# m-hamza-mughal/RAG-Gesture

Hardware: AMD Instinct MI355X
Metric: SMPL-X frames/sec, len150 DDIM-50 + insertion guidance; 1/2/4/8 GPU (higher is better)
Workload: dtype bf16

## Files before the change

include/rg_gesture.h:

```cpp
#ifndef RG_GESTURE_H
#define RG_GESTURE_H

#include <stdint.h>

#ifdef __cplusplus
extern "C" {
#endif

typedef struct rg_handle rg_handle;

enum rg_status {
  RG_OK = 0,
  RG_ERR_INVALID = -1,
  RG_ERR_HIP = -2,
  RG_ERR_NO_DEVICE = -3
};

#define RG_VERSION 127
int rg_version(void);
int rg_create(rg_handle** out, int device);
void rg_destroy(rg_handle* h);
const char* rg_last_error(rg_handle* h);
int rg_num_cus(rg_handle* h);

int rg_ddim_update(rg_handle* h, const float* x, const float* x0, float* x_out, int64_t n,
                   float c_recip, float c_recipm1, float c_a, float c_b, void* stream);

int rg_cfg_ddim_update(rg_handle* h, const float* out, const float* x, float* x_out, float* x0_out,
                       const float* js, int B, int T, int D, float w_c, float w_u,
                       float c_recip, float c_recipm1, float c_a, float c_b, void* stream);
int rg_cfg_ddim_update_rows(rg_handle* h, const float* out_cond, const float* out_uncond, const float* x, float* x_out,
                            float* x_out2, const float* js, int B, int T, int D, float w_c, float w_u,
                            float c_recip, float c_recipm1, float c_a, float c_b, void* stream);

int rg_cfg_ddpm_update(rg_handle* h, const float* out, const float* x, const float* noise, float* x_out,
                       const float* js, int B, int T, int D, float w_c, float w_u, float c1, float c2, float sigma,
                       void* stream);

typedef struct rg_glue_args {
  const float* out_c_a;
  const float* out_u_a;
// ... 159 lines not shown
  const float* tbias;
  const float* src_mask;
  const float* qmask;
  float* head;
  float* dump;
  float* xbuf;
  void* gbuf;
  const int* form;
  int L, B, T, S;
  int step, step_b, split;
  int dump_stage, dump_layer;
  int pairs;
  int twin;
  int* glue_ctr;
  rg_glue_args glue;
} rg_seq_args;

int rg_seq_forward(rg_handle* h, const rg_seq_args* args_host, void* stream);
int rg_seq2_forward(rg_handle* h, const rg_seq_args* args_host, void* stream);

#define RG_SEQ_MANY_MAX 8
int rg_seq_forward_many(rg_handle* h, const rg_seq_args* const* args_host, int n, void* stream);

#define RG_LANE_STRIDE 32
int rg_seqx_forward(rg_handle* h, const rg_seq_args* args_host, void* stream);
int rg_lane_form(rg_handle* h, int* state, int lane, int nlanes, int narrow_wgs, int wide_wgs, int budget, void* stream);

typedef struct rg_venc_args {
  const void* wstream;
  const void* pstream;
  const float* x;
  float* out;
  float* xbuf;
  float* dump;
  int nseq, S, nb, dump_block;
  const int* post_rows;
  float* post_mu;
  float* post_logvar;
  int post_nrows, pad_;
} rg_venc_args;

int rg_venc_forward(rg_handle* h, const rg_venc_args* args_host, void* stream);
int rg_venc_forward_grouped(rg_handle* h, const rg_venc_args* args_host, int n, void* stream);

typedef struct rg_vdec_args {
  const void* wstream;
// ... 473 lines not shown
```

rag-gesture_amd/csrc/rg_seq2.hip:

```cpp
#if !defined(RG_SEQ_BODY_ONLY) && !defined(RG2_PACK_TWO)
#define RG_PACK2_ONE
#endif
#include "rg_common.h"
#include "rg_stationary.h"
#include "rg_tail.h"
#include "rg_seq_host.h"

namespace {

constexpr int RD = 6;
constexpr int UPL = RG_SEQ_UPL;
constexpr int PANEL = TP * 1024;
constexpr int OFF_RING = 2 * PANEL;
constexpr int NSEG_COND = 36, NSEG_UNC = 19, NSEG_TWIN = 34;
constexpr int NSEG_MAX = NSEG_COND > NSEG_TWIN ? NSEG_COND : NSEG_TWIN;
constexpr int MAX_SEG = 8 * NSEG_MAX + 5;
constexpr int OFF_DESC = OFF_RING + NW * RD * 1024;
constexpr int OFF_STAT = OFF_DESC + ((MAX_SEG * 8 + 15) & ~15);
constexpr int STAT_HALF = 2 * NW * TP * 2;
constexpr int LDS_BYTES = OFF_STAT + 2 * STAT_HALF * 4;
static_assert(LDS_BYTES <= 160 * 1024, "LDS budget");

#define U(name) U_##name = RG_SEQ_U_##name
enum { U(KV), U(KV2), U(Q), U(SAO), U(MIXX), U(Q3_0), U(MIX_0), U(Q3_1), U(MIX_1), U(Q3_2), U(MIX_2), U(FF1_0), U(FF2_0), U(FF1_1), U(FF2_1), U(FFO) };
// ... 31 lines not shown
#else
#define TLOG()
#endif

typedef std::integral_constant<int, 3> SeqBoth;
typedef std::integral_constant<int, 1> SeqFirst;
typedef std::integral_constant<int, 2> SeqSecond;

typedef f32x4 Acc2[2][4][3];
typedef u32x2 Held[2][4][3];

__device__ __forceinline__ void zero(Acc2& a) {
#pragma unroll
  for (int q = 0; q < 2; ++q)
#pragma unroll
    for (int j = 0; j < 4; ++j)
#pragma unroll
      for (int tb = 0; tb < 3; ++tb) a[q][j][tb] = f32x4{0.f, 0.f, 0.f, 0.f};
}

}

template <bool TWIN>
__device__ __forceinline__ void run_pair(const rg_seq_args& a, const int sA, const int sB, unsigned char* const smem) {
  float* const sStat = reinterpret_cast<float*>(smem + OFF_STAT);
  int tid_ = threadIdx.x;
  asm volatile("" : "+v"(tid_));
  const int tid = tid_, lane0 = tid & 63;
  const int wave = __builtin_amdgcn_readfirstlane(tid >> 6);
  unsigned char* const ring = smem + OFF_RING + wave * (RD * 1024);
  const int T = a.T, B = a.B, L = a.L, R = 2 * a.B;
  const bool cond = sA < B;
  const int seqs[2] = {sA, sB};
  const int clips[2] = {cond ? sA : sA - B, (cond && !TWIN) ? sB : sB - B};
  const int st = clips[0] >= a.split ? a.step_b : a.step;
#ifdef RG_STAMPS
  unsigned long long tacc[12] = {0, 0, 0, 0, 0, 0, 0, 0, 0, 0, 0, 0};
  int ncall = 0;
  const unsigned long long tk0 = __builtin_amdgcn_s_memrealtime();
#endif
  auto barx = [&]() {
    TSTART();
    bar();
    TSTOP(2);
  };
  const int NU = UPL * L + 2;
  const int nspl = TWIN ? NSEG_TWIN : cond ? NSEG_COND : NSEG_UNC;
// ... 75 lines not shown
          u32x4{pack2(v0[0], v0[1]), pack2(v0[2], v0[3]), pack2(v1[0], v1[1]), pack2(v1[2], v1[3])};
    }
  __syncthreads();

  rg_cursor<RD, rg_desc8> cur(ring, smem + OFF_DESC, wave, lane0);
  auto ring_wait = [&]() { wait_vmcnt<RD - 1>(); };
  auto consume = [&]() -> const unsigned char* {
#ifdef RG_STAMPS
    const unsigned long long tc0_ = __builtin_amdgcn_s_memrealtime();
    ring_wait();
    tacc[7] += __builtin_amdgcn_s_memrealtime() - tc0_;
#else
    ring_wait();
#endif
    return ring + cur.head * 1024;
  };
  cur.load_seg();
#pragma unroll
  for (int s = 0; s < RD; ++s) cur.issue(s);
#ifdef RG_STAMPS
  tacc[10] = __builtin_amdgcn_s_memrealtime() - tk0;
#endif

  float* const Rw = a.xbuf + ((size_t)blockIdx.x * 2 * NW + wave) * (12 * 64 * 4);
  unsigned char* const Gw = reinterpret_cast<unsigned char*>(a.gbuf) + (size_t)blockIdx.x * (8 * PANEL);
  auto store_R = [&](const Acc2& v) {
    LANE_LOCAL();
    TSTART();
#pragma unroll
    for (int q = 0; q < 2; ++q)
#pragma unroll
      for (int j = 0; j < 4; ++j)
#pragma unroll
        for (int tb = 0; tb < 3; ++tb)
          *reinterpret_cast<f32x4*>(Rw + ((size_t)(q * NW * 12 + j * 3 + tb) * 64 + lane) * 4) = v[q][j][tb];
    TSTOP(6);
  };
  auto load_R = [&](Acc2& v) {
    LANE_LOCAL();
    TSTART();
#pragma unroll
    for (int q = 0; q < 2; ++q)
#pragma unroll
      for (int j = 0; j < 4; ++j)
#pragma unroll
        for (int tb = 0; tb < 3; ++tb)
          v[q][j][tb] = *reinterpret_cast<const f32x4*>(Rw + ((size_t)(q * NW * 12 + j * 3 + tb) * 64 + lane) * 4);
    TSTOP(6);
// ... 692 lines not shown
  const int npc = ((split + 1) >> 1) + ((B - split + 1) >> 1);
  return pairs ? npc : 2 * npc;
}
__device__ __forceinline__ void seq2_block(const rg_seq_args& a, const int block, unsigned char* const smem) {
  const int B = a.B, split = min(max(a.split, 0), B);
  const int npc = ((split + 1) >> 1) + ((B - split + 1) >> 1);
  int p = block, kind0 = 0;
  if (!a.pairs) {
    if ((npc & 3) == 0) {
      const int x = block & 7, q = block >> 3;
      kind0 = x >= 4;
      p = 4 * q + (x & 3);
    } else {
      kind0 = block >= npc;
      p = block - kind0 * npc;
    }
  }
  int c0, c1;
  pair_clips(p, split, B, c0, c1);
  const int npass = a.pairs ? 2 : 1;
#pragma unroll 1
  for (int pass = 0; pass < npass; ++pass) {
    const int kind = a.pairs ? pass : kind0;
    run_pair<false>(a, c0 + kind * B, c1 + kind * B, smem);
    __syncthreads();
    int* const ctr = rg_tail::late_ctr();
    if (ctr && !a.dump_stage)
      rg_tail::arrive_and_glue<NTH>(ctr, c0, c1, reinterpret_cast<int*>(smem), __builtin_amdgcn_readfirstlane(threadIdx.x >> 6));
  }
}

#ifndef RG_SEQ_BODY_ONLY
__global__ void __launch_bounds__(NTH) rg_seq2_kernel(const rg_seq_args a) {
  extern __shared__ __attribute__((aligned(16))) unsigned char smem[];
#ifndef RG2_SHARE_SIMD
  RG_OWN_THE_SIMD();
#endif
  seq2_block(a, blockIdx.x, smem);
}

__global__ void __launch_bounds__(NTH) rg_seq2_twin_kernel(const rg_seq_args a) {
  extern __shared__ __attribute__((aligned(16))) unsigned char smem[];
#ifndef RG2_SHARE_SIMD
  RG_OWN_THE_SIMD();
#endif
  const int clip = blockIdx.x;
  run_pair<true>(a, clip, clip + a.B, smem);
  __syncthreads();
  if (rg_tail::late_ctr() && !a.dump_stage) rg_tail::glue_own<NTH>(clip, __builtin_amdgcn_readfirstlane(threadIdx.x >> 6));
}

extern "C" int rg_seq2_forward(rg_handle* h, const rg_seq_args* args_host, void* stream) {
  const std::string why = rg_seq_refusal(RG_SEQ2_ENTRY, args_host);
  if (!why.empty()) { if (h) h->err = why; return RG_ERR_INVALID; }
  const rg_seq_args& a = *args_host;
  static rg_attr_once lds_once, lds_once_twin;
  if (a.twin) { RG_RESERVE_LDS(h, lds_once_twin, rg_seq2_twin_kernel, LDS_BYTES); }
  else { RG_RESERVE_LDS(h, lds_once, rg_seq2_kernel, LDS_BYTES); }
  rg_prof_scope prof(h, stream, 3, rg_seq_flops(a));
  if (a.twin) hipLaunchKernelGGL(rg_seq2_twin_kernel, dim3(a.B), dim3(NTH), LDS_BYTES, rg_stream(stream), a);
  else hipLaunchKernelGGL(rg_seq2_kernel, dim3(seq2_grid(a.B, a.split, a.pairs)), dim3(NTH), LDS_BYTES, rg_stream(stream), a);
  RG_CHECK_LAUNCH(h);
  prof.stop();
  return RG_OK;
}
#endif
```

rag-gesture_amd/csrc/rg_seq_host.h:

```cpp
#pragma once
#include <string>

#include "../../include/rg_gesture.h"

struct rg_seq_entry { const char *name, *need_bufs, *need_form, *no_dump, *twin_range, *twin_pairs, *no_twin; };
constexpr rg_seq_entry RG_SEQ_ENTRY = {"rg_seq_forward", nullptr, nullptr, nullptr, nullptr, nullptr, nullptr};
constexpr rg_seq_entry RG_SEQ2_ENTRY = {"rg_seq2_forward", "the two-sequence forward needs its scratch buffers xbuf and gbuf", nullptr,
                                        nullptr, "twin must be 0 or 1", "twin and pairs are two launch forms: set one of them", nullptr};
constexpr rg_seq_entry RG_SEQX_ENTRY = {
    "rg_seqx_forward", "the two-sequence form needs its scratch buffers xbuf and gbuf", "form: the lane's flag (rg_lane_form) must be given",
    "diagnostic dumps: use rg_seq_forward / rg_seq2_forward", nullptr, nullptr,
    "the twin form (one clip per workgroup) is not one of the device-chosen forms: use rg_seq2_forward"};

inline bool rg_seq_glue_ok(const rg_seq_args& a) {
  if (!a.glue_ctr) return true;
  const rg_glue_args& g = a.glue;
  if (a.dump_stage || g.n_a < 0 || g.n_b < 0 || g.n_a + g.n_b != a.B || g.T != a.T || g.D != 512 || !g.js || g.g_iter_next < 0) return false;
  if (g.n_a && !(g.out_c_a && g.out_u_a && g.x_a)) return false;
  if (g.n_b && !(g.out_c_b && g.out_u_b && g.x_b)) return false;
  return !g.in_seq_next || g.noise_next;
}

inline std::string rg_seq_refusal(const rg_seq_entry& e, const rg_seq_args* args) {
  const char* why = nullptr;
// ... 16 lines not shown
  }
  return why ? std::string(e.name) + ": " + why : std::string();
}

constexpr rg_seq_entry RG_SEQ_MANY_ENTRY = {"rg_seq_forward_many", nullptr, nullptr, "diagnostic dumps: use rg_seq_forward", nullptr, nullptr,
                                            "the twin form is rg_seq2_forward's: a grouped launch runs one workgroup per sequence"};

inline std::string rg_seq_many_refusal(const rg_seq_args* const* args, const int n) {
  const std::string name = std::string(RG_SEQ_MANY_ENTRY.name) + ": ";
  if (!args || n < 1) return name + "null or empty list of sessions";
  if (n > RG_SEQ_MANY_MAX) return name + "too many sessions (at most RG_SEQ_MANY_MAX)";
  for (int i = 0; i < n; ++i) {
    const std::string why = rg_seq_refusal(RG_SEQ_MANY_ENTRY, args[i]);
    if (!why.empty()) return why;
    const rg_seq_args &a = *args[i], &a0 = *args[0];
    if (a.pairs) return name + "pairs is another launch form: a grouped launch runs one workgroup per sequence";
    if (!(a.L == a0.L && a.T == a0.T && a.S == a0.S)) return name + "the sessions must agree in L, T and S";
    if (!(a.wstream == a0.wstream && a.pstream == a0.pstream && a.ustream == a0.ustream))
      return name + "the sessions must share the weight, parameter and table streams";
  }
  return std::string();
}

inline double rg_seq_flops(const rg_seq_args& a) {
  const double unit = 2.0 * a.T * 512 * 512, att = 2.0 * a.T * 32 * 32 * 16;
  const double cond = (RG_SEQ_UPL * a.L + 2) * unit + a.L * (2 + 3) * att, unc = (10 * a.L + 2) * unit + a.L * 2 * att;
  return a.B * (cond + unc);
}
```

rag-gesture_amd/csrc/rg_tail.h:

```cpp
#pragma once
#include "rg_common.h"
#include <cstddef>

namespace rg_tail {

typedef __attribute__((ext_vector_type(4))) float f32x4;
typedef __attribute__((ext_vector_type(4))) unsigned u32x4;
constexpr int COHERENT = 17;

__device__ __forceinline__ float ddim_one(float x, float x0, float c_recip, float c_recipm1, float c_a, float c_b) {
#pragma clang fp contract(off)
  float eps = (c_recip * x - x0) / c_recipm1;
  return x0 * c_a + c_b * eps;
}
__device__ __forceinline__ float cfg_one(float oc, float ou, float jc, float ju, float w_c, float w_u) {
#pragma clang fp contract(off)
  return oc * w_c * jc + ou * w_u * ju;
}

template <typename P>
__device__ __forceinline__ P* uniform_ptr(P* p) {
  const unsigned long long v = reinterpret_cast<unsigned long long>(p);
  return reinterpret_cast<P*>((unsigned long long)__builtin_amdgcn_readfirstlane((unsigned)(v >> 32)) << 32 |
                              (unsigned)__builtin_amdgcn_readfirstlane((unsigned)v));
// ... 153 lines not shown
  if (wave == 0 && lane == 0) {
    int m = 0;
    if (__hip_atomic_fetch_add(ctr + c0, 1, __ATOMIC_RELAXED, __HIP_MEMORY_SCOPE_AGENT) & 1) m |= 1;
    if (c1 != c0 && (__hip_atomic_fetch_add(ctr + c1, 1, __ATOMIC_RELAXED, __HIP_MEMORY_SCOPE_AGENT) & 1)) m |= 2;
    *flag = m;
  }
  __syncthreads();
  const int m = *flag;
  __syncthreads();
  if (m == 0) return;
  const rg_glue_args g = late_arg<rg_glue_args>(base + offsetof(rg_seq_args, glue));
  const float ton = two_over_numel(g);
#pragma unroll 1
  for (int q = 0; q < 2; ++q) {
    if (!(m >> q & 1)) continue;
    const int c = q ? c1 : c0;
    const bool ga = c < g.n_a;
    const int cl = ga ? c : c - g.n_a;
    glue_clip<NTH / 64>(g, ga, cl, wave, lane, ton);
  }
}

template <int NTH>
__device__ __forceinline__ void glue_own(const int c, const int wave) {
  const int lane = __builtin_amdgcn_mbcnt_hi(~0u, __builtin_amdgcn_mbcnt_lo(~0u, 0u));
  const rg_glue_args g = late_arg<rg_glue_args>(offsetof(rg_seq_args, glue));
  const bool ga = c < g.n_a;
  glue_clip<NTH / 64>(g, ga, ga ? c : c - g.n_a, wave, lane, two_over_numel(g));
}
}
```

rag-gesture_amd/denoiser.py:

```python
import math

import numpy as np
import torch

from . import capi, gemm as G, seqfwd as SQ

CONDS = ("xf_text", "xf_audio", "xf_spk")
BLOCKS = ("sa_block", "ca_blocks.xf_text", "ca_blocks.xf_audio", "ca_blocks.xf_spk", "ffn")


def _timestep_embedding(timesteps, dim, max_period=10000):
    half = dim // 2
    freqs = torch.exp(-math.log(max_period) * torch.arange(0, half, dtype=torch.float32) / half)
    args = timesteps[:, None].float() * freqs[None]
    return torch.cat([torch.cos(args), torch.sin(args)], dim=-1)


class DenoiserWeights:

    KV_GROUP = 2

    @staticmethod
    def _fold_ln(W, b, gamma, beta, pw, f32):
        Wp = (W.double() * gamma.double()[None, :]).float()
# ... 322 lines not shown
    def chain_end(self):
        if self.sq is not None:
            self.sq.chain_end()

    def forward(self, x, step, step_b=None, split=None, glue=None):
        w, h, B, R, M, D, T = self.w, self.h, self.B, self.R, self.M, self.w.D, self.w.T
        if split is not None and not (0 < split < B):
            step, step_b, split = (step if split >= B else step_b), None, None
        if self.sq is not None:
            if glue is not None and not x.is_contiguous():
                raise capi.RgError("DenoiserSession.forward(glue=...): x is updated in place and must be contiguous")
            return self.sq.run(x.contiguous(), step, step_b, split, glue=glue)
        if glue is not None:
            raise capi.RgError("DenoiserSession.forward(glue=...): the sequence-stationary engine only")
        if self.ln_mode == "auto":
            out = self._forward_guarded(x, step)
            if split is None:
                return out
        return self._forward_chain(x, step, step_b, split)

    @staticmethod
    def forward_many(sessions, calls):
        for s, kw in zip(sessions, calls):
            if s.sq is None or not kw["x"].is_contiguous():
                raise capi.RgError("DenoiserSession.forward_many: the sequence-stationary engine only, x contiguous")
        return SQ.run_many([s.sq for s in sessions], calls)

    LN_GUARD_SIGMAS = 3.0

    def _forward_guarded(self, x, step):
        if torch.cuda.is_current_stream_capturing():
            raise capi.RgError("DenoiserSession(ln_mode='auto'): run one forward before capturing a graph")
        self._guard = torch.zeros(1, device=self.w.dev)
        self.ln_mode = "folded"
        out = self._forward_chain(x, step)
        self.ln_ratio = float(self._guard.item())
        self._guard = None
        if self.ln_ratio > self.LN_GUARD_SIGMAS ** 2:
            self.ln_mode, self.xa_bf = "prologue", None
            out = self._forward_chain(x, step)
        return out

    def _guard_stats(self, stats):
        if getattr(self, "_guard", None) is not None:
            self.h.call("ln_guard", stats, self.M, stats.shape[1], self.w.D, self._guard)

# ... 118 lines not shown
```

rag-gesture_amd/pipeline.py:

```python
import collections
import ctypes
import contextlib
import copy
import os
import time
import types

import torch
import yaml

from . import capi, denoiser, sampler, schedule as sched_mod, seqfwd, vae as vae_mod

MODELS = {}


def register_module(cls):
    MODELS[cls.__name__] = cls
    return cls


def register_with_mmcv(force=False):
    regs = []
    try:
        from mmcv.cnn import MODELS as mmcv_models
# ... 42 lines not shown
        "step_increasing_from_25": list(range(steps - 1, -1, -1))[:half] + [0] * half,
        "decreasing_till_25": [0] * half + list(range(half)),
        "increasing_from_25": list(range(half - 1, -1, -1)) + [0] * half,
    }
    if name not in table:
        raise ValueError("Invalid guidance_iters value")
    return table[name]


E_BUCKET = 4


def bucket(n, m=None):
    m = E_BUCKET if m is None else m
    return -(-n // m) * m


def pad_rows(t, n):
    return t if t.shape[0] == n else torch.cat([t, t[:1].expand(n - t.shape[0], *t.shape[1:])], dim=0)


def lane_rows(t, dim, b0, b1):
    return None if t is None else (t[b0:b1] if dim == 0 else t[:, b0:b1])


def exemplar_query_masks(qmask, clips, n):
    return {c: pad_rows(torch.stack([qmask[b] for b in clips]), n) for c in denoiser.CONDS}


class _TorchNoise:
    order_free = True

    def __init__(self, device, generator=None):
        self.device, self.generator = device, generator

    def draw(self, shape, device=None):
        return torch.randn(*shape, device=self.device, generator=self.generator)


def draw_batch_noise(tape, dev, B, T, D, S, use_inversion, use_insertion_guidance, visualize_inversion, ddpm, has_in_seq, n_exemplars):
    x = tape.draw((B, T, D)).to(dev).contiguous()
    start_noise = x if use_inversion else None
    invl = torch.zeros(S, B, T, D, device=dev) if use_inversion and use_insertion_guidance else None
    ddpm_noise = inseq_noise = None
    if use_inversion and visualize_inversion and not isinstance(tape, _TorchNoise):
        for _ in range(S * sum(n_exemplars[:B])):
# ... 166 lines not shown
        return {k: copy.deepcopy(v, memo) for k, v in dict.items(self) if k not in self._PLAIN}

    def __reduce__(self):
        self._ready()
        return (dict, (), None, None, iter([(k, v) for k, v in dict.items(self) if k not in self._PLAIN]))


@register_module
class MotionDiffusion(torch.nn.Module):

    profile_phases = False
    rotation_lanes = None
    form_lanes = None
    _cur_rot = None
    _last_state = None

    def __init__(self, model=None, loss_recon=None, loss_gen=None, loss_contact=None, loss_laplace=None,
                 diffusion_train=None, diffusion_test=None, init_cfg=None, inference_type="ddpm",
                 genloss_acceleration_weight=True, genloss_hands_weight=2, genloss_smooth=True,
                 body_part_lossweights=None, device="cuda", precision="bf16", lanes=2, sample_lanes=None, session_options=None,
                 vae_options=None, async_results=False, slots=2, max_inflight=2, cobatch_lanes="batch", base_lanes=8,
                 batch_lanes=4, lane_streams=None, calibrate_lanes=True, decode_stream=False, dynamic_forms=False, dynamic_budget=None, invert_alone_wide=True, tail_glue=True,
                 cache_exemplar_latents=True, exemplar_cache_bytes=8 << 30, skip_clip_encode=True, grouped_decode=True,
                 grouped_drain=True, **kwargs):
        super().__init__()
        self.grouped_drain = bool(grouped_drain)
        self.grouped_decode = bool(grouped_decode)
        self.cache_exemplar_latents, self.exemplar_cache_bytes = bool(cache_exemplar_latents), int(exemplar_cache_bytes)
        self.skip_clip_encode = bool(skip_clip_encode)
        self.model = build_submodule(model, device=device, **kwargs)
        dt = dict(diffusion_test)
        self.schedule = sched_mod.Schedule(beta_scheduler=dt["beta_scheduler"], diffusion_steps=dt["diffusion_steps"],
                                           respace=dt.get("respace"))
        capi.require(dt.get("model_mean_type", "start_x") == "start_x" and dt.get("classifier_free_guidance_scale", 0) == 0,
                "unsupported argument: requires dt.get(\"model_mean_type\", \"start_x\") == \"start_x\" and dt.get(\"classifier_free_guidance_scale\", 0) == 0")
        self.inference_type = inference_type
        capi.require(inference_type in ("ddim", "ddpm"), "inference_type is 'ddim' (shipped config) or 'ddpm'")
        self.device, self.precision = torch.device(device), precision
        self.training = False
        self.session_options, self.vae_options = dict(session_options or {}), dict(vae_options or {})
        self.vae_options.setdefault("grouped_decode", self.grouped_decode)
        self._state = None
        self._sessions = {}
        self._graphs = {}
        self.use_graphs = True
        self.graph_captures = self.graph_cross_stream_waits = 0
        self._jitter = None
        self.phase_ms = {}
# ... 356 lines not shown
        motion_mask = gre.latent_mask(kwargs["motion_mask"].float())
        T = motion_mask.shape[1]
        n_lat = (T - 3) // 4
        up_i, ha_i, fa_i, lt_i = (list(range(0, n_lat)), list(range(n_lat + 1, 2 * n_lat + 1)),
                                  list(range(2 * n_lat + 2, 3 * n_lat + 2)), list(range(3 * n_lat + 3, T)))
        qmask = torch.ones_like(motion_mask)
        for r in ((T - 3) // 4, 2 * (T - 3) // 4, 3 * (T - 3) // 4):
            qmask[:, r] = 0
        query_masks = {c: qmask for c in denoiser.CONDS}

        plan = self._lane_plan(B)
        plan_s = self._lane_plan(B, self.sample_lanes)
        main = torch.cuda.current_stream()
        run_async = self.async_results and self.slots > 1 and not self.profile_phases
        cob = self._cob if run_async else None
        pid = None
        if cob is not None and cob.get("lane") is not None:
            self._lane_plan(B)
            n_rot = self.rotation_lanes or (self.batch_lanes if use_inversion else self.base_lanes)
            n_rot = max(1, min(int(n_rot), len(self._lane_streams)))
            self._cur_rot = self.form_lanes or n_rot
            pid = cob["lane"] % n_rot
            plan = plan_s = [(pid, self._lane_streams[pid], 0, B)]
        if run_async:
            self._slot = self._take_slot(pid, main, self._lanes_of(plan, plan_s))
        else:
            self._slot = 0
            self._wait_slot(main, self._lanes_of(plan, plan_s), 0)
        gre.concurrent_parts(not run_async and not self.use_graphs)
        word, audio, spk = kwargs["word"], kwargs["audio"], kwargs["speaker_ids"]
        with self._phase("conditions"):
            for lane, stream, b0, b1 in ([] if cob is not None else plan_s):
                cstream = main if run_async else stream
                cstream.wait_stream(main)
                with torch.cuda.stream(cstream):
                    self._sample_conditions(lane, b0, b1, word, audio, spk, motion_mask, qmask)
        with self._phase("vae_encode"):
            if self.skip_clip_encode and not self.training:
                tr_rel = gre.relative_trans(kwargs["motion_upper"], kwargs["motion_lower"], kwargs["motion_face"],
                                            kwargs["motion_hands"], f(kwargs["trans"]))
                capi.require(4 * (kwargs["motion_upper"].shape[1] // gre.frame_chunk_size) + 3 == T,
                             "unsupported argument: requires motion.shape[1] == T")
            else:
                motion, tr_rel = gre.encode_device_graphed(
                    f(kwargs["motion_upper"]), f(kwargs["motion_lower"]), f(kwargs["motion_face"]), f(kwargs["motion_hands"]),
                    f(kwargs["trans"]), f(kwargs["facial"]), f(kwargs["contact"]), [f(e) for e in eps_list])
                capi.require(motion.shape[1] == T, "unsupported argument: requires motion.shape[1] == T")
# ... 127 lines not shown

    def flush(self):
        cob, self._cob = self._cob, dict(lane=0)
        try:
            self._finish_pending()
        finally:
            self._cob = cob
        out = list(self._ready)
        self._ready.clear()
        return out

    def _finish_alone(self, st):
        main = st.main = torch.cuda.current_stream()
        st.slot = self._take_slot(st.pid, main, self._lanes_of(st.plan_s))
        for lane, stream, b0, b1 in st.plan_s:
            self._sample_conditions(lane, b0, b1, st.word, st.audio, st.spk, st.motion_mask, st.qmask)
        self._sampling_pass(st)
        return self._tail(st)

    def _pending_upto(self, seq):
        return sorted((p for p in self._pend if self._pend[p].seq <= seq), key=lambda p: self._pend[p].seq)

    def _finish_pending(self, upto=None, resume=None):
        sts = [self._pend.pop(p) for p in self._pending_upto(float("inf") if upto is None else upto)]
        group = self._drain_group(sts) if self.grouped_drain else []
        if group:
            self._drain_grouped(group)
        for st in sts:
            self._ready.append(self._tail(st) if any(st is g for g in group) else self._finish_alone(st))
        if resume is not None:
            self._slot = self._slots[resume.pid] = resume.slot

    DRAIN_SLOT = 0

    def _drain_group(self, sts):
        sett = lambda st: (st.T, st.S, bool(st.use_insertion_guidance), tuple(int(v) for v in st.guidance_iters), float(st.guidance_lr))

        def alone_on_a_lane(st):
            return (st.run_async and st.via_submit and not st.ddpm and st.prev_future is None and st.plan == st.plan_s
                    and len(st.plan_s) == 1 and tuple(st.plan_s[0][2:]) == (0, st.B))

        def one_sequence_form(st):
            o = self._session_opts(st.B, "sample", st.plan_s[0][0])
            return (self._runs_seq_engine(o) and not o.get("seq_pairs") and not o.get("seq_duo") and not o["seq_twin"] and "lane_dyn" not in o
                    and o["tail_glue"] and sampler.TAIL_GLUE and self.model.weights.h.recorder is None)
        if self.precision != "bf16":
# ... 46 lines not shown
        ins = {}
        for tag, (word, audio, spk, mask, qm) in (("a", a), ("b", b)):
            ins["word_" + tag], ins["audio_" + tag] = word.to(dev).float(), audio.to(dev).float()
            ins["spk_" + tag], ins["mask_" + tag] = spk.to(dev).long(), mask.to(dev).float()
            for c in denoiser.CONDS:
                ins["q_%s_%s" % (c, tag)] = qm[c].to(dev).float()

        def run(st):
            for tag, off, fin in (("a", 0, False), ("b", n_a, True)):
                sess.set_conditions(st["word_" + tag], st["audio_" + tag], st["spk_" + tag], st["mask_" + tag],
                                    {c: st["q_%s_%s" % (c, tag)] for c in denoiser.CONDS}, offset=off, finalize=fin)
            return ()
        self._graph_run(key + tuple(tuple(v.shape) for v in ins.values()), ins, run, owner=own)

    def _submit_chain(self, st):
        pend, S, T, D, dev = self._pend.get(st.pid), st.S, st.T, st.D, self.device
        lanes = [(lane, stream, b0, b1, self._exemplars(st, b0, b1)) for lane, stream, b0, b1 in st.plan] if st.use_inversion else []
        so = self.session_options
        groups_ok = self.precision == "bf16" and (self._runs_seq_engine(so) or so.get("styl_prepass", True))
        can_defer = (groups_ok and st.use_inversion and not st.visualize_inversion and not st.ddpm and st.plan == st.plan_s
                     and all(ex for *_, ex in lanes))
        same = pend is not None and can_defer and (pend.B, pend.T) == (st.B, st.T) and \
            [(b0, b1) for _, _, b0, b1 in pend.plan] == [(b0, b1) for _, _, b0, b1 in st.plan]
        if pend is not None and not same:
            self._finish_pending(pend.seq, resume=st)
            pend = None
        if not can_defer:
            self._finish_pending(resume=st)
            for lane, stream, b0, b1 in st.plan_s:
                self._sample_conditions(lane, b0, b1, st.word, st.audio, st.spk, st.motion_mask, st.qmask)
            self._inversion_pass(st)
            self._sampling_pass(st)
            self._ready.append(self._tail(st))
            return None
        if pend is None:
            self._inversion_pass(st)
            for lane, stream, _, _ in st.plan:
                self._slot_done[(lane, st.slot)] = [stream.record_event()]
            self._pend[st.pid] = st
            return None
        main = st.main
        self._fill_prev(pend, main)
        guided = pend.use_insertion_guidance
        gi, lr = tuple(int(v) for v in pend.guidance_iters), float(pend.guidance_lr)
        work = []
        for lane, stream, b0, b1, ex in lanes:
            Bl = b1 - b0
            Ep, cat = self._exemplar_inputs(st, ex, main)
            okey = (Bl + Ep, "cobatch", lane, self._slot)
            sess = self._session(Bl + Ep, "cobatch", lane)
            eqm = exemplar_query_masks(st.qmask, [b for b, _ in ex], Ep)
            self._set_conditions_pair(
                sess, ("cond2", Bl, Ep, lane, self._slot), okey,
                (pend.word[b0:b1], pend.audio[b0:b1], pend.spk[b0:b1], pend.motion_mask[b0:b1], {c: pend.qmask[b0:b1] for c in denoiser.CONDS}),
                (cat("retr_text"), cat("retr_audio"), cat("retr_spkid"), cat("retr_motion_mask"), eqm), Bl)
            work.append((lane, stream, b0, b1, ex, Ep, sess, okey, cat("retr_motion_latent").float().contiguous()))
        for lane, stream, b0, b1, ex, Ep, sess, okey, x_e in work:
            Bl = b1 - b0
            stream.wait_stream(main)
            self._used_on(stream, pend.x, pend.in_seq, pend.inseq_noise, pend.invl, pend.x_out, x_e, st.start_noise, st.invl, st.qmask)
            with torch.cuda.stream(stream):
                sl = lambda t, dim: lane_rows(t, dim, b0, b1)
                ins = dict(xa=sl(pend.x, 0), in_seq=sl(pend.in_seq, 0), noise=sl(pend.inseq_noise, 1),
                           invl=sl(pend.invl, 1) if guided else None, xb=x_e)

                def loop(s, sess=sess, Bl=Bl, Ep=Ep):
                    x_all = torch.cat([s["xa"], s["xb"]], dim=0).contiguous()
                    out_b = torch.empty(S, Ep, T, D, device=dev)
                    sampler.cobatched_loop(sess, x_all, Bl, out_b, inverted_a=s["invl"], guidance_iters=gi, guidance_lr=lr,
                                           inseq_noise_a=s["noise"], in_seq_a=s["in_seq"], tail_glue=self.tail_glue)
                    return x_all[:Bl], out_b
                key = ("cobatch", Bl, Ep, lane, T, self._slot, guided, pend.in_seq is not None, gi, lr, self.tail_glue)
                xl, inv = self._graph_run(key, ins, loop, owner=okey)
                pend.x_out[b0:b1].copy_(xl)
                self._splice(st, ex, inv, Ep)
                self._zero_prev_rows(st, b0, b1)
        pend.main, pend.slot = main, self._slot
        self._ready.append(self._tail(pend))
        self._pend[st.pid] = st
        return None

    def _exemplars(self, st, b0, b1):
        return [(b, q) for b in range(b0, b1) for q in st.retrieval_dict["retr_uncropped_latents"][b].keys()]

    def _exemplar_inputs(self, st, ex, stream):
        dev = self.device
        Ep = bucket(len(ex))
        lat = lambda b, q: st.retrieval_dict["retr_uncropped_latents"][b][q]

        def cat(key):
            parts = [lat(b, q)[key].to(dev) for b, q in ex]
            self._used_on(stream, *parts)
            return pad_rows(torch.cat(parts, dim=0), Ep)
        return Ep, cat

    def _splice(self, st, ex, inv, Ep):
        h, rd = self.model.weights.h, st.retrieval_dict
        lvl = st.inversion_start_time % st.S
        rows = []
        for e, (b, q_idx) in enumerate(ex):
            r0, r1 = rd["retr_startends"][b][q_idx]
            q0, q1 = rd["query_startends"][b][q_idx]
            capi.require(r1 - r0 == q1 - q0, "unsupported argument: requires r1 - r0 == q1 - q0")
# ... 136 lines not shown
```

rag-gesture_amd/sampler.py:

```python
import ctypes

import torch

from . import capi

from .seqfwd import GlueArgs, MANY_MAX

SPLICE_MAX = capi.header_constants()["RG_SPLICE_MAX"]
SpliceTable = capi.struct("rg_splice_table")


TAIL_GLUE = True


def _tail_ok(sess, x):
    return (TAIL_GLUE and getattr(sess, "tail_glue", True) and getattr(sess, "sq", None) is not None and sess.h.recorder is None and x.is_cuda and x.is_contiguous()
            and x.dtype == torch.float32 and x.shape[0] == sess.B)


def _p(t):
    if t is None:
        return None
    if not (t.is_cuda and t.is_contiguous() and t.dtype == torch.float32):
        raise capi.RgError("rg_cobatch_glue: contiguous fp32 device tensors expected")
# ... 138 lines not shown
        tail = bool(tail_glue) and _tail_ok(sess, x_all) and 0 < n_a < B
        for k in range(S):
            i = S - 1 - k
            if not tail:
                sess.forward(x_all, i, step_b=k, split=n_a)
            nxt = None if i == 0 else (inverted_a[i - 1] if inverted_a is not None else in_seq_a)
            a = _glue(sess, guidance_lr, i=i, x_a=xa, n_a=n_a, nxt=nxt, noise_nxt=None if nxt is None else inseq_noise_a[i - 1],
                      g_next=guidance_iters[i - 1] if inverted_a is not None and i > 0 else 0, k=k, x_b=xb, keep_b=out_b[k], n_b=n_b)
            if tail:
                sess.forward(x_all, i, step_b=k, split=n_a, glue=a)
            else:
                h.call("cobatch_glue", ctypes.byref(a))
        sess.chain_end()
        return x_all, out_b
    for k in range(S):
        i, g_iter = S - 1 - k, None
        if inverted_a is not None and i != S - 1:
            in_seq, g_iter = inverted_a[i], guidance_iters[i]
        _step(sess, xa, i, in_seq, None if in_seq is None else inseq_noise_a[i], g_iter, guidance_lr, n_a, (x_all, k, xb, out_b[k]))
    sess.chain_end()
    return x_all, out_b


class GraphedLoop:

    def __init__(self, fn, warmup=True):
        if warmup:
            s = torch.cuda.Stream()
            s.wait_stream(torch.cuda.current_stream())
            with torch.cuda.stream(s):
                fn()
            torch.cuda.current_stream().wait_stream(s)
        self.graph = torch.cuda.CUDAGraph()
        with capi.capture(self.graph):
            fn()

    def replay(self):
        self.graph.replay()
```

rag-gesture_amd/seqfwd.py:

```python
import ctypes

import torch

from . import capi

_C = capi.header_constants()
UPL = _C["RG_SEQ_UPL"]
(U_KV, U_KV2, U_Q, U_SAO, U_MIXX, U_Q3_0, U_MIX_0, U_Q3_1, U_MIX_1, U_Q3_2, U_MIX_2, U_FF1_0, U_FF2_0, U_FF1_1, U_FF2_1, U_FFO) = (
    _C["RG_SEQ_U_" + n] for n in "KV KV2 Q SAO MIXX Q3_0 MIX_0 Q3_1 MIX_1 Q3_2 MIX_2 FF1_0 FF2_0 FF1_1 FF2_1 FFO".split())
CONDS = ("xf_text", "xf_audio", "xf_spk")
LANE_STRIDE = _C["RG_LANE_STRIDE"]
GlueArgs = capi.struct("rg_glue_args")
SeqArgs = capi.struct("rg_seq_args")


def supported(cfg, T, precision):
    return (precision == "bf16" and cfg["latent_dim"] == 512 and cfg["num_heads"] == 16 and cfg["ff_size"] == 1024
            and T <= 48 and 1 <= cfg["num_layers"] <= 8)


def pack_unit(W):
    capi.require(W.shape == (512, 512), "unsupported argument: requires W.shape == (512, 512)")
    v = W.to(torch.bfloat16).view(8, 4, 16, 16, 4, 8)
    return v.permute(0, 3, 1, 4, 2, 5).contiguous().view(8, 64, 64, 8)
# ... 144 lines not shown
        a.dump = dump.data_ptr() if dump is not None else None
        a.dump_stage, a.dump_layer = int(dump_stage), int(dump_layer)
        return a

    def run(self, x, step, step_b=None, split=None, dump=None, dump_stage=0, dump_layer=0, glue=None):
        a = self._set_args(x, step, step_b, split, dump, dump_stage, dump_layer, glue)
        if self.lane_dyn is not None and not dump_stage:
            state, lane, n, budget = self.lane_dyn
            B = self.sess.B
            wide = 2 * B
            if self.duo:
                sp = max(0, min(B, a.split))
                npc = (sp + 1) // 2 + (B - sp + 1) // 2
                narrow = npc if a.pairs else 2 * npc
            else:
                narrow = wide = B if a.pairs else 2 * B
            self.h.call("lane_form", state, lane, n, narrow, wide, budget)
        self.h.call("seq2_forward" if dump_stage and self.lane_dyn is not None and self.duo else self._entry, ctypes.byref(a))
        return self.sess.head

    def groupable(self):
        return not self.duo and not self.twin and not self.args.pairs and self.lane_dyn is None

    def chain_end(self):
        if self.lane_dyn is not None:
            state, lane, n, budget = self.lane_dyn
            self.h.call("lane_form", state, lane, n, 0, 0, budget)


MANY_MAX = _C["RG_SEQ_MANY_MAX"]


def run_many(sqs, calls):
    if not (1 <= len(sqs) <= MANY_MAX and len(sqs) == len(calls)):
        raise capi.RgError("rg_seq_forward_many: 1 to %d sessions, one set of arguments each" % MANY_MAX)
    if not all(sq.groupable() for sq in sqs):
        raise capi.RgError("rg_seq_forward_many: sessions in the one-workgroup-per-sequence form only (no duo, pairs, twin or lane_dyn)")
    args = [sq._set_args(**kw) for sq, kw in zip(sqs, calls)]
    ptrs = (ctypes.c_void_p * len(args))(*[ctypes.addressof(a) for a in args])
    sqs[0].h.call("seq_forward_many", ctypes.cast(ptrs, ctypes.c_void_p), len(args))
    return [sq.sess.head for sq in sqs]
```

Measured before the change: 70660.

## Group parked twin-form cobatch chains into one multi-session seq2 launch per step

Adds a grouped twin-form kernel that runs up to eight sessions' clips in a single launch, with per-session arguments packed into the kernarg block and the per-workgroup scratch indexed by clip instead of blockIdx. The pipeline now parks compatible guided cobatch chains from different lanes and runs them together as one captured graph that calls the grouped kernel each DDIM step. The aim is to fill the GPU better and cut launch and graph count for small per-lane batches. The cost is added scheduling complexity: deferred slot assignment, parking windows and flushes, and extra graph-cache keys per lane combination.

Result: faster. 80010 (median of 6 runs) (+13.2%).

```diff
diff --git a/include/rg_gesture.h b/include/rg_gesture.h
--- a/include/rg_gesture.h
+++ b/include/rg_gesture.h
@@ -16,7 +16,7 @@
   RG_ERR_NO_DEVICE = -3
 };
 
-#define RG_VERSION 127
+#define RG_VERSION 128
 int rg_version(void);
 int rg_create(rg_handle** out, int device);
 void rg_destroy(rg_handle* h);
@@ -222,6 +222,8 @@
 #define RG_SEQ_MANY_MAX 8
 int rg_seq_forward_many(rg_handle* h, const rg_seq_args* const* args_host, int n, void* stream);
 
+int rg_seq2_forward_many(rg_handle* h, const rg_seq_args* const* args_host, int n, void* stream);
+
 #define RG_LANE_STRIDE 32
 int rg_seqx_forward(rg_handle* h, const rg_seq_args* args_host, void* stream);
 int rg_lane_form(rg_handle* h, int* state, int lane, int nlanes, int narrow_wgs, int wide_wgs, int budget, void* stream);
diff --git a/profiles/chain_captures.py b/profiles/chain_captures.py
--- /dev/null
+++ b/profiles/chain_captures.py
@@ -0,0 +1,35 @@
+import importlib
+import os
+import sys
+
+ROOT = os.path.dirname(os.path.dirname(os.path.abspath(__file__)))
+sys.path.insert(0, ROOT)
+os.environ.setdefault("GPU_MAX_HW_QUEUES", "2")
+rg = importlib.import_module("rag-gesture_amd")
+import torch
+import bench
+
+bench.torch = torch
+
+steps = int(sys.argv[1]) if len(sys.argv) > 1 else 20
+warmup = int(sys.argv[2]) if len(sys.argv) > 2 else 2
+dev = torch.device("cuda", 0)
+wl = bench.Workload(rg, "guided", 16, dev, 0, 32768, clips=16)
+m = wl.model
+wl.prime()
+torch.cuda.synchronize()
+print("options %s: grouped_chains %s" % (os.environ.get("RG_BENCH_MODEL_KWARGS", "{}"), m.grouped_chains))
+print("after prime():            graph_captures %d, graphs in the cache %d" % (m.graph_captures, len(m._graphs)), flush=True)
+for _ in range(warmup):
+    wl.step()
+wl.drain()
+torch.cuda.synchronize()
+print("after %d warm-up steps:     graph_captures %d" % (warmup, m.graph_captures), flush=True)
+before = m.graph_captures
+for _ in range(steps):
+    wl.step()
+wl.drain()
+torch.cuda.synchronize()
+print("after %d timed steps:      graph_captures %d (%d captured in the timed steps)" % (steps, m.graph_captures, m.graph_captures - before))
+keys = sorted({k[0] for k in m._graphs})
+print("graph kinds: " + ", ".join("%s x%d" % (k, sum(1 for g in m._graphs if g[0] == k)) for k in keys))
diff --git a/profiles/twin_many_time.py b/profiles/twin_many_time.py
--- /dev/null
+++ b/profiles/twin_many_time.py
@@ -0,0 +1,65 @@
+import importlib
+import os
+import sys
+
+sys.path.insert(0, os.path.dirname(os.path.dirname(os.path.abspath(__file__))))
+import torch
+
+rg = importlib.import_module("rag-gesture_amd")
+from oracle import denoiser as od
+
+B, NA, T, N, REPS = 64, 16, 43, 4, 20
+cfg = rg.synth.default_model_cfg(num_layers=8)
+W = rg.denoiser.DenoiserWeights(rg.synth.synth_denoiser_state(0, cfg), cfg, rg.schedule.Schedule(), "cuda")
+mm = torch.ones(B, T)
+mm[:, [10, 21, 32]] = 0
+sessions, xs = [], []
+for k in range(N):
+    data = rg.synth.synth_batch(B, seed=3 + k)
+    sess = rg.denoiser.DenoiserSession(W, B, engine="seq", seq_duo=True, seq_twin=True)
+    sess.set_conditions(data["word"], data["audio"], data["speaker_ids"], mm, od.make_query_masks(mm))
+    sessions.append(sess)
+    xs.append(torch.randn(B, T, 512, device="cuda"))
+many = rg.denoiser.DenoiserSession.forward_many
+
+
+def fn_all(fn, streams):
+    if not streams:
+        fn(None)
+    for i, s in enumerate(streams):
+        with torch.cuda.stream(s):
+            fn(i)
+
+
+def timed(fn, streams=()):
+    cur = torch.cuda.current_stream()
+    for _ in range(3):
+        fn_all(fn, streams)
+    torch.cuda.synchronize()
+    e0, e1 = torch.cuda.Event(enable_timing=True), torch.cuda.Event(enable_timing=True)
+    e0.record()
+    for s in streams:
+        s.wait_stream(cur)
+    for _ in range(REPS):
+        fn_all(fn, streams)
+    for s in streams:
+        cur.wait_stream(s)
+    e1.record()
+    torch.cuda.synchronize()
+    return e0.elapsed_time(e1) * 1e3 / REPS
+
+
+print("rg_seq2_forward_many, sessions of %d clips (%d + %d), L = 8, T = %d, %d launches per figure" % (B, NA, B - NA, T, REPS))
+for n in (1, 2, 4):
+    calls = [dict(x=xs[k], step=20, step_b=30, split=NA) for k in range(n)]
+    for rep in range(3):
+        us = timed(lambda _: many(sessions[:n], [dict(c) for c in calls]))
+        print("grouped  n=%d (%3d workgroups) run %d: %8.1f us per launch, %7.1f us per session" % (n, n * B, rep, us, us / n), flush=True)
+one = lambda i: sessions[i or 0].forward(xs[i or 0], 20, 30, NA)
+for rep in range(3):
+    us = timed(one)
+    print("rg_seq2_forward alone (64 workgroups)   run %d: %8.1f us per launch" % (rep, us), flush=True)
+streams = [torch.cuda.Stream(), torch.cuda.Stream()]
+for rep in range(3):
+    us = timed(one, streams)
+    print("two lanes, one session each (2 x 64)    run %d: %8.1f us per pair of launches, %7.1f us per session" % (rep, us, us / 2), flush=True)
diff --git a/rag-gesture_amd/csrc/rg_seq2.hip b/rag-gesture_amd/csrc/rg_seq2.hip
--- a/rag-gesture_amd/csrc/rg_seq2.hip
+++ b/rag-gesture_amd/csrc/rg_seq2.hip
@@ -77,7 +77,7 @@
 }
 
 template <bool TWIN>
-__device__ __forceinline__ void run_pair(const rg_seq_args& a, const int sA, const int sB, unsigned char* const smem) {
+__device__ __forceinline__ void run_pair(const rg_seq_args& a, const int sA, const int sB, const int wg, unsigned char* const smem) {
   float* const sStat = reinterpret_cast<float*>(smem + OFF_STAT);
   int tid_ = threadIdx.x;
   asm volatile("" : "+v"(tid_));
@@ -199,8 +199,8 @@
   tacc[10] = __builtin_amdgcn_s_memrealtime() - tk0;
 #endif
 
-  float* const Rw = a.xbuf + ((size_t)blockIdx.x * 2 * NW + wave) * (12 * 64 * 4);
-  unsigned char* const Gw = reinterpret_cast<unsigned char*>(a.gbuf) + (size_t)blockIdx.x * (8 * PANEL);
+  float* const Rw = a.xbuf + ((size_t)(unsigned)wg * 2 * NW + wave) * (12 * 64 * 4);
+  unsigned char* const Gw = reinterpret_cast<unsigned char*>(a.gbuf) + (size_t)(unsigned)wg * (8 * PANEL);
   auto store_R = [&](const Acc2& v) {
     LANE_LOCAL();
     TSTART();
@@ -939,7 +939,7 @@
 #pragma unroll 1
   for (int pass = 0; pass < npass; ++pass) {
     const int kind = a.pairs ? pass : kind0;
-    run_pair<false>(a, c0 + kind * B, c1 + kind * B, smem);
+    run_pair<false>(a, c0 + kind * B, c1 + kind * B, block, smem);
     __syncthreads();
     int* const ctr = rg_tail::late_ctr();
     if (ctr && !a.dump_stage)
@@ -962,7 +962,7 @@
   RG_OWN_THE_SIMD();
 #endif
   const int clip = blockIdx.x;
-  run_pair<true>(a, clip, clip + a.B, smem);
+  run_pair<true>(a, clip, clip + a.B, clip, smem);
   __syncthreads();
   if (rg_tail::late_ctr() && !a.dump_stage) rg_tail::glue_own<NTH>(clip, __builtin_amdgcn_readfirstlane(threadIdx.x >> 6));
 }
@@ -981,4 +981,50 @@
   prof.stop();
   return RG_OK;
 }
+
+struct rg_seq2_many_block {
+  rg_seq_args a[RG_SEQ_MANY_MAX];
+  int end[RG_SEQ_MANY_MAX];
+};
+static_assert(sizeof(rg_seq2_many_block) <= 4096, "the parameter block must fit the kernarg segment");
+
+__global__ void __launch_bounds__(NTH) rg_seq2_twin_many_kernel(const rg_seq2_many_block p) {
+  extern __shared__ __attribute__((aligned(16))) unsigned char smem[];
+  RG_OWN_THE_SIMD();
+  const int block = blockIdx.x;
+  int s = 0, first = 0;
+#pragma unroll
+  for (int i = 0; i + 1 < RG_SEQ_MANY_MAX; ++i)
+    if (block >= p.end[i]) { s = i + 1; first = p.end[i]; }
+  s = __builtin_amdgcn_readfirstlane(s);
+  const int clip = block - first;
+  const rg_seq_args& a = p.a[s];
+  run_pair<true>(a, clip, clip + a.B, clip, smem);
+  __syncthreads();
+  const unsigned base = (unsigned)(offsetof(rg_seq2_many_block, a) + s * sizeof(rg_seq_args));
+  if (rg_tail::late_ctr(base) && !a.dump_stage) rg_tail::glue_own<NTH>(clip, __builtin_amdgcn_readfirstlane(threadIdx.x >> 6), base);
+}
+
+extern "C" int rg_seq2_forward_many(rg_handle* h, const rg_seq_args* const* args_host, int n, void* stream) {
+  const std::string why = rg_seq2_many_refusal(args_host, n);
+  if (!why.empty()) { if (h) h->err = why; return RG_ERR_INVALID; }
+  rg_seq2_many_block p{};
+  int total = 0;
+  double flops = 0.0;
+  for (int i = 0; i < RG_SEQ_MANY_MAX; ++i) {
+    if (i < n) {
+      p.a[i] = *args_host[i];
+      total += p.a[i].B;
+      flops += rg_seq_flops(p.a[i]);
+    }
+    p.end[i] = total;
+  }
+  static rg_attr_once lds_once;
+  RG_RESERVE_LDS(h, lds_once, rg_seq2_twin_many_kernel, LDS_BYTES);
+  rg_prof_scope prof(h, stream, 3, flops);
+  hipLaunchKernelGGL(rg_seq2_twin_many_kernel, dim3(total), dim3(NTH), LDS_BYTES, rg_stream(stream), p);
+  RG_CHECK_LAUNCH(h);
+  prof.stop();
+  return RG_OK;
+}
 #endif
diff --git a/rag-gesture_amd/csrc/rg_seq_host.h b/rag-gesture_amd/csrc/rg_seq_host.h
--- a/rag-gesture_amd/csrc/rg_seq_host.h
+++ b/rag-gesture_amd/csrc/rg_seq_host.h
@@ -62,6 +62,25 @@
   return std::string();
 }
 
+constexpr rg_seq_entry RG_SEQ2_MANY_ENTRY = {"rg_seq2_forward_many", RG_SEQ2_ENTRY.need_bufs, nullptr, "diagnostic dumps: use rg_seq2_forward",
+                                             RG_SEQ2_ENTRY.twin_range, RG_SEQ2_ENTRY.twin_pairs, nullptr};
+
+inline std::string rg_seq2_many_refusal(const rg_seq_args* const* args, const int n) {
+  const std::string name = std::string(RG_SEQ2_MANY_ENTRY.name) + ": ";
+  if (!args || n < 1) return name + "null or empty list of sessions";
+  if (n > RG_SEQ_MANY_MAX) return name + "too many sessions (at most RG_SEQ_MANY_MAX)";
+  for (int i = 0; i < n; ++i) {
+    const std::string why = rg_seq_refusal(RG_SEQ2_MANY_ENTRY, args[i]);
+    if (!why.empty()) return why;
+    const rg_seq_args &a = *args[i], &a0 = *args[0];
+    if (!a.twin) return name + "every session must be in the twin form (twin == 1): a grouped launch runs one workgroup per clip";
+    if (!(a.L == a0.L && a.T == a0.T && a.S == a0.S)) return name + "the sessions must agree in L, T and S";
+    if (!(a.wstream == a0.wstream && a.pstream == a0.pstream && a.ustream == a0.ustream))
+      return name + "the sessions must share the weight, parameter and table streams";
+  }
+  return std::string();
+}
+
 inline double rg_seq_flops(const rg_seq_args& a) {
   const double unit = 2.0 * a.T * 512 * 512, att = 2.0 * a.T * 32 * 32 * 16;
   const double cond = (RG_SEQ_UPL * a.L + 2) * unit + a.L * (2 + 3) * att, unc = (10 * a.L + 2) * unit + a.L * 2 * att;
diff --git a/rag-gesture_amd/csrc/rg_tail.h b/rag-gesture_amd/csrc/rg_tail.h
--- a/rag-gesture_amd/csrc/rg_tail.h
+++ b/rag-gesture_amd/csrc/rg_tail.h
@@ -199,9 +199,9 @@
 }
 
 template <int NTH>
-__device__ __forceinline__ void glue_own(const int c, const int wave) {
+__device__ __forceinline__ void glue_own(const int c, const int wave, const unsigned base = 0) {
   const int lane = __builtin_amdgcn_mbcnt_hi(~0u, __builtin_amdgcn_mbcnt_lo(~0u, 0u));
-  const rg_glue_args g = late_arg<rg_glue_args>(offsetof(rg_seq_args, glue));
+  const rg_glue_args g = late_arg<rg_glue_args>(base + offsetof(rg_seq_args, glue));
   const bool ga = c < g.n_a;
   glue_clip<NTH / 64>(g, ga, ga ? c : c - g.n_a, wave, lane, two_over_numel(g));
 }
diff --git a/rag-gesture_amd/denoiser.py b/rag-gesture_amd/denoiser.py
--- a/rag-gesture_amd/denoiser.py
+++ b/rag-gesture_amd/denoiser.py
@@ -368,6 +368,9 @@
     @staticmethod
     def forward_many(sessions, calls):
         for s, kw in zip(sessions, calls):
+            sp = kw.get("split")
+            if sp is not None and not (0 < sp < s.B):
+                kw["step"], kw["step_b"], kw["split"] = (kw["step"] if sp >= s.B else kw["step_b"]), None, None
             if s.sq is None or not kw["x"].is_contiguous():
                 raise capi.RgError("DenoiserSession.forward_many: the sequence-stationary engine only, x contiguous")
         return SQ.run_many([s.sq for s in sessions], calls)
diff --git a/rag-gesture_amd/pipeline.py b/rag-gesture_amd/pipeline.py
--- a/rag-gesture_amd/pipeline.py
+++ b/rag-gesture_amd/pipeline.py
@@ -88,6 +88,10 @@
 
 def lane_rows(t, dim, b0, b1):
     return None if t is None else (t[b0:b1] if dim == 0 else t[:, b0:b1])
+
+
+def window_accepts(parked, new, size):
+    return len(parked) < size and all(lane != new[0] and (sett, rot) == (new[1], new[2]) for lane, sett, rot in parked)
 
 
 def exemplar_query_masks(qmask, clips, n):
@@ -300,8 +304,9 @@
                  vae_options=None, async_results=False, slots=2, max_inflight=2, cobatch_lanes="batch", base_lanes=8,
                  batch_lanes=4, lane_streams=None, calibrate_lanes=True, decode_stream=False, dynamic_forms=False, dynamic_budget=None, invert_alone_wide=True, tail_glue=True,
                  cache_exemplar_latents=True, exemplar_cache_bytes=8 << 30, skip_clip_encode=True, grouped_decode=True,
-                 grouped_drain=True, **kwargs):
+                 grouped_drain=True, grouped_chains=True, **kwargs):
         super().__init__()
+        self.grouped_chains, self._parked, self._win, self._n_rot = bool(grouped_chains), [], 0, 1
         self.grouped_drain = bool(grouped_drain)
         self.grouped_decode = bool(grouped_decode)
         self.cache_exemplar_latents, self.exemplar_cache_bytes = bool(cache_exemplar_latents), int(exemplar_cache_bytes)
@@ -704,7 +709,16 @@
             self._cur_rot = self.form_lanes or n_rot
             pid = cob["lane"] % n_rot
             plan = plan_s = [(pid, self._lane_streams[pid], 0, B)]
-        if run_async:
+            if self._parked and (n_rot != self._n_rot or not use_inversion):
+                self._launch_parked()
+            self._n_rot = n_rot
+        elif self._parked:
+            self._launch_parked()
+        slot_later = (run_async and pid is not None and self.grouped_chains and use_inversion and self._pend.get(pid) is not None
+                      and not self.profile_phases)
+        if slot_later:
+            self._slot = None
+        elif run_async:
             self._slot = self._take_slot(pid, main, self._lanes_of(plan, plan_s))
         else:
             self._slot = 0
@@ -878,6 +892,7 @@
         return sorted((p for p in self._pend if self._pend[p].seq <= seq), key=lambda p: self._pend[p].seq)
 
     def _finish_pending(self, upto=None, resume=None):
+        self._launch_parked()
         sts = [self._pend.pop(p) for p in self._pending_upto(float("inf") if upto is None else upto)]
         group = self._drain_group(sts) if self.grouped_drain else []
         if group:
@@ -970,6 +985,12 @@
                      and all(ex for *_, ex in lanes))
         same = pend is not None and can_defer and (pend.B, pend.T) == (st.B, st.T) and \
             [(b0, b1) for _, _, b0, b1 in pend.plan] == [(b0, b1) for _, _, b0, b1 in st.plan]
+        park = same and self._can_park(st, pend, lanes)
+        if self._parked and not (park and self._joins_parked(st, pend)):
+            self._launch_parked(resume=st)
+        if st.slot is None:
+            lane_set = self._lanes_of(st.plan, st.plan_s)
+            st.slot = self._take_slot(st.pid, st.main, lane_set, slot=self._win % self.slots if park else None)
         if pend is not None and not same:
             self._finish_pending(pend.seq, resume=st)
             pend = None
@@ -1003,6 +1024,23 @@
                 (pend.word[b0:b1], pend.audio[b0:b1], pend.spk[b0:b1], pend.motion_mask[b0:b1], {c: pend.qmask[b0:b1] for c in denoiser.CONDS}),
                 (cat("retr_text"), cat("retr_audio"), cat("retr_spkid"), cat("retr_motion_mask"), eqm), Bl)
             work.append((lane, stream, b0, b1, ex, Ep, sess, okey, cat("retr_motion_latent").float().contiguous()))
+        if park:
+            self._parked.append(types.SimpleNamespace(st=st, pend=pend, work=work, slot=self._slot, lane=work[0][0], n_rot=self._n_rot,
+                                                      sett=self._chain_settings(st, pend)))
+            self._pend[st.pid] = st
+            if len(self._parked) >= min(self._n_rot, self.CHAIN_GROUP):
+                self._launch_parked(resume=st)
+            return None
+        self._chain_alone(st, pend, work, main)
+        pend.main, pend.slot = main, self._slot
+        self._ready.append(self._tail(pend))
+        self._pend[st.pid] = st
+        return None
+
+    def _chain_alone(self, st, pend, work, main):
+        S, T, D, dev = st.S, st.T, st.D, self.device
+        guided = pend.use_insertion_guidance
+        gi, lr = tuple(int(v) for v in pend.guidance_iters), float(pend.guidance_lr)
         for lane, stream, b0, b1, ex, Ep, sess, okey, x_e in work:
             Bl = b1 - b0
             stream.wait_stream(main)
@@ -1023,10 +1061,94 @@
                 pend.x_out[b0:b1].copy_(xl)
                 self._splice(st, ex, inv, Ep)
                 self._zero_prev_rows(st, b0, b1)
-        pend.main, pend.slot = main, self._slot
-        self._ready.append(self._tail(pend))
-        self._pend[st.pid] = st
-        return None
+
+    CHAIN_GROUP = 4
+
+    @staticmethod
+    def _chain_settings(st, pend):
+        return (st.T, st.S, bool(pend.use_insertion_guidance), tuple(int(v) for v in pend.guidance_iters), float(pend.guidance_lr))
+
+    def _can_park(self, st, pend, lanes):
+        if not (self.grouped_chains and self.precision == "bf16" and st.run_async and st.via_submit and st.pid is not None
+                and pend.prev_future is None and len(lanes) == 1 and tuple(lanes[0][2:4]) == (0, st.B)
+                and min(self._n_rot, self.CHAIN_GROUP, sampler.MANY_MAX) >= 2
+                and self.tail_glue and sampler.TAIL_GLUE and self.model.weights.h.recorder is None):
+            return False
+        lane, ex = lanes[0][0], lanes[0][4]
+        return self._twin_tail_form(self._session_opts(st.B + bucket(len(ex)), "cobatch", lane))
+
+    def _twin_tail_form(self, o):
+        return bool(self._runs_seq_engine(o) and o.get("seq_twin") and o.get("seq_duo") and not o.get("seq_pairs")
+                    and "lane_dyn" not in o and o.get("tail_glue"))
+
+    def _joins_parked(self, st, pend):
+        return window_accepts([(r.lane, r.sett, r.n_rot) for r in self._parked], (st.pid, self._chain_settings(st, pend), self._n_rot),
+                              min(self._n_rot, self.CHAIN_GROUP))
+
+    def _launch_parked(self, resume=None):
+        recs, self._parked = self._parked, []
+        if not recs:
+            return
+        main = torch.cuda.current_stream()
+        cob, self._cob = self._cob, self._cob or dict(lane=0)
+        try:
+            if len(recs) == 1:
+                r = recs[0]
+                self._slot = r.slot
+                self._chain_alone(r.st, r.pend, r.work, main)
+            else:
+                self._chains_grouped(recs, main)
+                self._win += 1
+            for r in recs:
+                r.pend.main, r.pend.slot = main, r.slot
+                self._ready.append(self._tail(r.pend))
+        finally:
+            self._cob = cob
+        if resume is not None and resume.slot is not None:
+            self._slot = self._slots[resume.pid] = resume.slot
+
+    def _chains_grouped(self, recs, main):
+        order = sorted(recs, key=lambda r: r.lane)
+        S, T, D, dev = order[0].st.S, order[0].st.T, order[0].st.D, self.device
+        _, _, guided, gi, lr = order[0].sett
+        g = order[0].work[0][1]
+        g.wait_stream(main)
+        ins, sessions, shapes = {}, [], []
+        for j, r in enumerate(order):
+            lane, stream, b0, b1, ex, Ep, sess, okey, x_e = r.work[0]
+            pend, st = r.pend, r.st
+            if stream is not g:
+                g.wait_stream(stream)
+            self._used_on(g, pend.x, pend.in_seq, pend.inseq_noise, pend.invl, pend.x_out, x_e, st.start_noise, st.invl, st.qmask)
+            ins.update({"xa%d" % j: pend.x, "in_seq%d" % j: pend.in_seq, "noise%d" % j: pend.inseq_noise,
+                        "invl%d" % j: pend.invl if guided else None, "xb%d" % j: x_e})
+            sessions.append(sess)
+            shapes.append((b1 - b0, Ep))
+        n = len(order)
+
+        def loop(s):
+            x_alls = [torch.cat([s["xa%d" % j], s["xb%d" % j]], dim=0).contiguous() for j in range(n)]
+            out_bs = [torch.empty(S, Ep, T, D, device=dev) for _, Ep in shapes]
+            sampler.cobatched_loop_many(sessions, x_alls, [Bl for Bl, _ in shapes], out_bs,
+                                        inverted_as=[s["invl%d" % j] for j in range(n)], guidance_iters=gi, guidance_lr=lr,
+                                        inseq_noise_as=[s["noise%d" % j] for j in range(n)], in_seq_as=[s["in_seq%d" % j] for j in range(n)],
+                                        tail_glue=self.tail_glue)
+            return tuple(t for j in range(n) for t in (x_alls[j][:shapes[j][0]], out_bs[j]))
+        owners = tuple(r.work[0][7] for r in order)
+        key = ("cobatch_many", owners, T, guided, tuple(r.pend.in_seq is not None for r in order), gi, lr, self.tail_glue)
+        with torch.cuda.stream(g):
+            outs = self._graph_run(key, ins, loop, owner=owners)
+        for j, r in enumerate(order):
+            lane, stream, b0, b1, ex, Ep, sess, okey, x_e = r.work[0]
+            xl, inv = outs[2 * j], outs[2 * j + 1]
+            if stream is not g:
+                stream.wait_stream(g)
+            self._used_on(stream, xl, inv)
+            with torch.cuda.stream(stream):
+                r.pend.x_out[b0:b1].copy_(xl)
+                self._splice(r.st, ex, inv, Ep)
+                self._zero_prev_rows(r.st, b0, b1)
+            r.pend.wait_streams = [g]
 
     def _exemplars(self, st, b0, b1):
         return [(b, q) for b in range(b0, b1) for q in st.retrieval_dict["retr_uncropped_latents"][b].keys()]
diff --git a/rag-gesture_amd/sampler.py b/rag-gesture_amd/sampler.py
--- a/rag-gesture_amd/sampler.py
+++ b/rag-gesture_amd/sampler.py
@@ -184,6 +184,42 @@
     return x_all, out_b
 
 
+def cobatched_many_ok(sessions, x_alls, n_as):
+    return (1 < len(sessions) <= MANY_MAX and all(_tail_ok(s, x) and s.sq.groupable_twin() and 0 < n < s.B for s, x, n in zip(sessions, x_alls, n_as))
+            and all(s.w is sessions[0].w for s in sessions) and len({id(s) for s in sessions}) == len(sessions))
+
+
+def cobatched_loop_many(sessions, x_alls, n_as, out_bs, inverted_as=None, guidance_iters=None, guidance_lr=0.1, inseq_noise_as=None,
+                        in_seq_as=None, tail_glue=True):
+    n = len(sessions)
+    none = [None] * n
+    inverted_as = none if inverted_as is None else inverted_as
+    inseq_noise_as = none if inseq_noise_as is None else inseq_noise_as
+    in_seq_as = none if in_seq_as is None else in_seq_as
+    if not (tail_glue and cobatched_many_ok(sessions, x_alls, n_as)):
+        for j in range(n):
+            cobatched_loop(sessions[j], x_alls[j], n_as[j], out_bs[j], inverted_a=inverted_as[j], guidance_iters=guidance_iters,
+                           guidance_lr=guidance_lr, inseq_noise_a=inseq_noise_as[j], in_seq_a=in_seq_as[j], tail_glue=tail_glue)
+        return x_alls, out_bs
+    S = sessions[0].w.schedule.num_timesteps
+    for j, sess in enumerate(sessions):
+        _insert_first(sess, x_alls[j][:n_as[j]], n_as[j], in_seq_as[j], inseq_noise_as[j])
+    for k in range(S):
+        i = S - 1 - k
+        calls = []
+        for j, sess in enumerate(sessions):
+            n_a = n_as[j]
+            nxt = None if i == 0 else (inverted_as[j][i - 1] if inverted_as[j] is not None else in_seq_as[j])
+            calls.append(dict(x=x_alls[j], step=i, step_b=k, split=n_a, glue=_glue(
+                sess, guidance_lr, i=i, x_a=x_alls[j][:n_a], n_a=n_a, nxt=nxt, noise_nxt=None if nxt is None else inseq_noise_as[j][i - 1],
+                g_next=guidance_iters[i - 1] if inverted_as[j] is not None and i > 0 else 0, k=k, x_b=x_alls[j][n_a:], keep_b=out_bs[j][k],
+                n_b=sess.B - n_a)))
+        type(sessions[0]).forward_many(sessions, calls)
+    for sess in sessions:
+        sess.chain_end()
+    return x_alls, out_bs
+
+
 class GraphedLoop:
 
     def __init__(self, fn, warmup=True):
diff --git a/rag-gesture_amd/seqfwd.py b/rag-gesture_amd/seqfwd.py
--- a/rag-gesture_amd/seqfwd.py
+++ b/rag-gesture_amd/seqfwd.py
@@ -190,6 +190,9 @@
     def groupable(self):
         return not self.duo and not self.twin and not self.args.pairs and self.lane_dyn is None
 
+    def groupable_twin(self):
+        return self.duo and self.twin and not self.args.pairs and self.lane_dyn is None
+
     def chain_end(self):
         if self.lane_dyn is not None:
             state, lane, n, budget = self.lane_dyn
@@ -202,9 +205,11 @@
 def run_many(sqs, calls):
     if not (1 <= len(sqs) <= MANY_MAX and len(sqs) == len(calls)):
         raise capi.RgError("rg_seq_forward_many: 1 to %d sessions, one set of arguments each" % MANY_MAX)
-    if not all(sq.groupable() for sq in sqs):
-        raise capi.RgError("rg_seq_forward_many: sessions in the one-workgroup-per-sequence form only (no duo, pairs, twin or lane_dyn)")
+    twin = all(sq.groupable_twin() for sq in sqs)
+    if not twin and not all(sq.groupable() for sq in sqs):
+        raise capi.RgError("rg_seq_forward_many: sessions in the one-workgroup-per-sequence form only (no duo, pairs, twin or lane_dyn), "
+                           "or all in the twin form (rg_seq2_forward_many)")
     args = [sq._set_args(**kw) for sq, kw in zip(sqs, calls)]
     ptrs = (ctypes.c_void_p * len(args))(*[ctypes.addressof(a) for a in args])
-    sqs[0].h.call("seq_forward_many", ctypes.cast(ptrs, ctypes.c_void_p), len(args))
+    sqs[0].h.call("seq2_forward_many" if twin else "seq_forward_many", ctypes.cast(ptrs, ctypes.c_void_p), len(args))
     return [sq.sess.head for sq in sqs]
```
